# arpg/vicalib

Hardware: AMD Instinct MI355X
Metric: corner_residuals_per_sec (higher is better)
Workload: dtype f64

## Files before the change

vicalib_amd/csrc/vc_imu.hpp:

```cpp
#pragma once
#include "vc_math.hpp"

namespace vc {

struct D1 { double a, v; };
VC_HD D1 mk(double a, double v = 0.0) { D1 r; r.a = a; r.v = v; return r; }
VC_HD D1 operator+(D1 x, D1 y) { return mk(x.a + y.a, x.v + y.v); }
VC_HD D1 operator-(D1 x, D1 y) { return mk(x.a - y.a, x.v - y.v); }
VC_HD D1 operator-(D1 x) { return mk(-x.a, -x.v); }
VC_HD D1 operator*(D1 x, D1 y) { return mk(x.a * y.a, x.a * y.v + x.v * y.a); }
VC_HD D1 operator/(D1 x, D1 y) { const double inv = fast_rcp(y.a), q = x.a * inv; return mk(q, (x.v - q * y.v) * inv); }
VC_HD D1 operator+(D1 x, double s) { return mk(x.a + s, x.v); }
VC_HD D1 operator+(double s, D1 x) { return mk(x.a + s, x.v); }
VC_HD D1 operator-(D1 x, double s) { return mk(x.a - s, x.v); }
VC_HD D1 operator-(double s, D1 x) { return mk(s - x.a, -x.v); }
VC_HD D1 operator*(D1 x, double s) { return mk(x.a * s, x.v * s); }
VC_HD D1 operator*(double s, D1 x) { return mk(x.a * s, x.v * s); }
VC_HD D1 operator/(D1 x, double s) { const double inv = 1.0 / s; return mk(x.a * inv, x.v * inv); }
VC_HD D1 operator/(double s, D1 y) { const double inv = fast_rcp(y.a); return mk(s * inv, -s * inv * inv * y.v); }
VC_HD bool operator<(D1 x, double y) { return x.a < y; }
VC_HD bool operator>(D1 x, double y) { return x.a > y; }
VC_HD D1 sqrt(D1 x) { double s, is; fast_sqrt_rsqrt(x.a, &s, &is); return mk(s, 0.5 * x.v * is); }
VC_HD D1 sin(D1 x) { return mk(::sin(x.a), ::cos(x.a) * x.v); }
VC_HD D1 cos(D1 x) { return mk(::cos(x.a), -::sin(x.a) * x.v); }
// ... 229 lines not shown
  imu_integrate_pose(*s, k, dt * 0.5, &y);
  imu_pose_derivative(y, g_w, z0, z1, par, dt / 2.0, k);
  for (int i = 0; i < 9; ++i) ks[i] = ks[i] + 2.0 * k[i];
  imu_integrate_pose(*s, k, dt, &y);
  imu_pose_derivative(y, g_w, z0, z1, par, dt, k);
  for (int i = 0; i < 9; ++i) k[i] = ks[i] + k[i];
  imu_integrate_pose(*s, k, dt / 6.0, &y);
  *s = y;
}
template <class T> VC_HD void imu_rk4_step(PoseV<T>* s, const Meas<T>& z0, const Meas<T>& z1, const T* b, const T* sf, const T* g_w) {
  const ImuParamsPtr<T> par = {b, sf};
  imu_rk4_step_p(s, z0, z1, par, g_w);
}
template <class T> VC_HD void imu_gravity(const T* dir, T* out) {
  const double g = 9.8007;
  const T sp = sin(dir[0]), cp = cos(dir[0]), sq = sin(dir[1]), cq = cos(dir[1]);
  out[0] = (cp * sq) * (-g);
  out[1] = (-1.0 * sp) * (-g);
  out[2] = (cp * cq) * (-g);
}

VC_HD void imu_gravity_record(const double* gdir, double* rec9) {
  for (int c = 0; c < 2; ++c) {
    const D1 d[2] = {mk(gdir[0], c == 0 ? 1.0 : 0.0), mk(gdir[1], c == 1 ? 1.0 : 0.0)};
    D1 g[3];
    imu_gravity(d, g);
    for (int i = 0; i < 3; ++i) { rec9[i] = g[i].a; rec9[3 + 3 * c + i] = g[i].v; }
  }
}
template <class T>
VC_HD void imu_residual_tail(const PoseV<T>& s, const double* w_sqrt, int rotation_only, const T* T2, const T* v2, T* r) {
  T qc[4] = {-T2[0], -T2[1], -T2[2], T2[3]};
  T nt[3] = {T2[4] * -1.0, T2[5] * -1.0, T2[6] * -1.0}, ti[3];
  tq_rotate(qc, nt, ti);
  T rel[7], tr[3];
  tq_mul(s.q, qc, rel);
  const T nrm = sqrt(rel[0] * rel[0] + rel[1] * rel[1] + rel[2] * rel[2] + rel[3] * rel[3]);
  for (int i = 0; i < 4; ++i) rel[i] = rel[i] / nrm;
  tq_rotate(s.q, ti, tr);
  for (int i = 0; i < 3; ++i) rel[4 + i] = s.p[i] + tr[i];
  T raw[9];
  tse3_log(rel, raw);
  for (int i = 0; i < 3; ++i) raw[6 + i] = s.v[i] - v2[i];
  for (int j = 0; j < 9; ++j) {
    T acc = cst<T>(0.0);
    for (int i = 0; i < 9; ++i) acc = acc + raw[i] * w_sqrt[i * 9 + j];
    r[j] = acc;
  }
  if (rotation_only) for (int i = 0; i < 3; ++i) { r[i] = cst<T>(0.0); r[6 + i] = cst<T>(0.0); }
}

template <class T>
VC_HD void imu_residual(const ImuView& buf, double t_start, double t_end, const double* w_sqrt, int rotation_only,
                        const T* T2, const T* T1, const T* v2, const T* v1, const T* gdir, const T* b, const T* sf, T toff, T* r) {
  const ImuRange rg = imu_range(buf, t_start, t_end, val(toff));
  if (!rg.valid) { for (int i = 0; i < 9; ++i) r[i] = cst<T>(0.0); return; }
  T gw[3];
  imu_gravity(gdir, gw);
  PoseV<T> s;
  for (int i = 0; i < 4; ++i) s.q[i] = T1[i];
  for (int i = 0; i < 3; ++i) { s.p[i] = T1[4 + i]; s.v[i] = v1[i]; }
  const int n_meas = (rg.k1 - rg.k0 + 1) + 2;
  Meas<T> z0, z1;
  imu_range_get(buf, rg, toff, t_start, t_end, 0, &z0);
  for (int m = 1; m < n_meas; ++m) {
    imu_range_get(buf, rg, toff, t_start, t_end, m, &z1);
    imu_rk4_step(&s, z0, z1, b, sf, gw);
    z0 = z1;
  }
  imu_residual_tail(s, w_sqrt, rotation_only, T2, v2, r);
}

VC_HD void local_jac_se3(const double* x, double* J) {
  for (int i = 0; i < 42; ++i) J[i] = 0.0;
  const double q1 = x[0], q2 = x[1], q3 = x[2], q0 = x[3];
  J[0 * 6 + 3] = 0.5 * q0; J[0 * 6 + 4] = -0.5 * q3; J[0 * 6 + 5] = 0.5 * q2;
  J[1 * 6 + 3] = 0.5 * q3; J[1 * 6 + 4] = 0.5 * q0; J[1 * 6 + 5] = -0.5 * q1;
  J[2 * 6 + 3] = -0.5 * q2; J[2 * 6 + 4] = 0.5 * q1; J[2 * 6 + 5] = 0.5 * q0;
  J[3 * 6 + 3] = -0.5 * q1; J[3 * 6 + 4] = -0.5 * q2; J[3 * 6 + 5] = -0.5 * q3;
  J[4 * 6 + 0] = 1.0 - 2.0 * (q2 * q2 + q3 * q3); J[4 * 6 + 1] = 2.0 * (q1 * q2 - q0 * q3); J[4 * 6 + 2] = 2.0 * (q1 * q3 + q0 * q2);
  J[5 * 6 + 0] = 2.0 * (q1 * q2 + q0 * q3); J[5 * 6 + 1] = 1.0 - 2.0 * (q1 * q1 + q3 * q3); J[5 * 6 + 2] = 2.0 * (q2 * q3 - q0 * q1);
  J[6 * 6 + 0] = 2.0 * (q1 * q3 - q0 * q2); J[6 * 6 + 1] = 2.0 * (q2 * q3 + q0 * q1); J[6 * 6 + 2] = 1.0 - 2.0 * (q1 * q1 + q2 * q2);
}

VC_HD void imu_block_direction(const ImuView& buf, double t_start, double t_end, const double* w_sqrt, int rotation_only,
                               const double* T2, const double* T1, const double* v2, const double* v1, const double* gdir,
                               const double* b, const double* sf, double toff, int dir, double* r, double* dr) {
  D1 P[35];
  for (int i = 0; i < 7; ++i) { P[i] = mk(T2[i]); P[7 + i] = mk(T1[i]); }
  for (int i = 0; i < 3; ++i) { P[14 + i] = mk(v2[i]); P[17 + i] = mk(v1[i]); }
  P[20] = mk(gdir[0]); P[21] = mk(gdir[1]);
  for (int i = 0; i < 6; ++i) { P[22 + i] = mk(b[i]); P[28 + i] = mk(sf[i]); }
  P[34] = mk(toff);
  for (int i = 0; i < 35; ++i) P[i].v = (i == dir) ? 1.0 : 0.0;
  D1 res[9];
  imu_residual<D1>(buf, t_start, t_end, w_sqrt, rotation_only, P, P + 7, P + 14, P + 17, P + 20, P + 22, P + 28, P[34], res);
  for (int i = 0; i < 9; ++i) { r[i] = res[i].a; dr[i] = res[i].v; }
}

constexpr int kDeltaCols = 14;

template <class T> struct DeltaAcc { T q[4], p[3], v[3], t; };
template <class T> VC_HD void imu_delta_append(DeltaAcc<T>* A, const PoseV<T>& d, T dt) {
  T rp[3], rv[3], q[4];
  tq_rotate(A->q, d.p, rp);
  tq_rotate(A->q, d.v, rv);
  tq_mul(A->q, d.q, q);
  for (int i = 0; i < 3; ++i) {
    A->p[i] = (A->p[i] + A->v[i] * dt) + rp[i];
    A->v[i] = A->v[i] + rv[i];
  }
  for (int i = 0; i < 4; ++i) A->q[i] = q[i];
  A->t = A->t + dt;
}
template <class T> VC_HD void imu_delta_then(DeltaAcc<T>* a, const DeltaAcc<T>& x) {
  PoseV<T> d;
  for (int k = 0; k < 4; ++k) d.q[k] = x.q[k];
  for (int k = 0; k < 3; ++k) { d.p[k] = x.p[k]; d.v[k] = x.v[k]; }
  imu_delta_append(a, d, x.t);
}
template <class T> VC_HD void imu_delta_identity(DeltaAcc<T>* a) {
  for (int k = 0; k < 3; ++k) { a->q[k] = cst<T>(0.0); a->p[k] = cst<T>(0.0); a->v[k] = cst<T>(0.0); }
  a->q[3] = cst<T>(1.0); a->t = cst<T>(0.0);
}
constexpr int kBlockDeltaStride = kDeltaCols * 11;

VC_HD void so3_exp_jl(const double* w, double* q, double* A, double* B) {
  const double th2 = w[0] * w[0] + w[1] * w[1] + w[2] * w[2];
  double imag, real;
  tso3_exp_factors(th2, &imag, &real);
  q[0] = imag * w[0]; q[1] = imag * w[1]; q[2] = imag * w[2]; q[3] = real;
  const bool tiny = th2 < 1e-6;
  *A = 2.0 * imag * imag;
  *B = tiny ? 1.0 / 6.0 - th2 * (1.0 / 120.0) : (1.0 - 2.0 * imag * real) * fast_rcp(tiny ? 1.0 : th2);
}
VC_HD void cross3(const double* a, const double* b, double* o) {
  const double x = a[1] * b[2] - a[2] * b[1], y = a[2] * b[0] - a[0] * b[2], z = a[0] * b[1] - a[1] * b[0];
  o[0] = x; o[1] = y; o[2] = z;
}
VC_HD void so3_jl_apply(const double* w, double A, double B, const double* d, double* o) {
  double c1[3], c2[3];
  cross3(w, d, c1);
  cross3(w, c1, c2);
  for (int i = 0; i < 3; ++i) o[i] = d[i] + A * c1[i] + B * c2[i];
}
VC_HD void mat3_vec(const double* R, const double* v, double* o) {
  const double a = R[0] * v[0] + R[1] * v[1] + R[2] * v[2];
  const double b = R[3] * v[0] + R[4] * v[1] + R[5] * v[2];
  const double c = R[6] * v[0] + R[7] * v[1] + R[8] * v[2];
  o[0] = a; o[1] = b; o[2] = c;
}
struct IntervalDeltaT { DeltaAcc<double> d; double dth[3], dp[3], dv[3], dt; double ap[3], av[3]; };
constexpr int kDtDoubles = 27;
VC_HD void imu_delta_t_identity(IntervalDeltaT* X) {
  imu_delta_identity(&X->d);
  for (int i = 0; i < 3; ++i) { X->dth[i] = 0.0; X->dp[i] = 0.0; X->dv[i] = 0.0; X->ap[i] = 0.0; X->av[i] = 0.0; }
  X->dt = 0.0;
}
VC_HD void imu_interval_delta_t(const ImuView& buf, const ImuRange& rg, D1 off, double t_start, double t_end, int m, int n_int,
                                const double* b, const double* sf, int gsel, IntervalDeltaT* X) {
  imu_delta_t_identity(X);
  const int kk = gsel < 3 ? gsel : (gsel < 6 ? gsel - 3 : 0);
  const bool seeded = gsel < 6, scale = gsel >= 3;
  double u0[3], u1[3], a0[3], a1[3], du0[3], du1[3], da0[3], da1[3], h, dh;
  double c0, c1;
  {
    Meas<D1> z0, z1;
    for (int k = 0; k < 3; ++k) { z0.w[k] = z0.a[k] = z1.w[k] = z1.a[k] = mk(0.0); }
    z0.time = z1.time = mk(0.0);
    if (m <= n_int) { imu_range_get_flat(buf, rg, off, t_start, t_end, m - 1, &z0); imu_range_get_flat(buf, rg, off, t_start, t_end, m, &z1); }
    if (z1.time.a == z0.time.a) return;
    h = z1.time.a - z0.time.a; dh = z1.time.v - z0.time.v;
    for (int i = 0; i < 3; ++i) {
      const double s0 = (seeded && i == kk) ? (scale ? z0.w[i].a : 1.0) : 0.0, s1 = (seeded && i == kk) ? (scale ? z1.w[i].a : 1.0) : 0.0;
      u0[i] = z0.w[i].a * sf[i] + b[i]; du0[i] = z0.w[i].v * sf[i] + s0;
      u1[i] = z1.w[i].a * sf[i] + b[i]; du1[i] = z1.w[i].v * sf[i] + s1;
      a0[i] = z0.a[i].a * sf[3 + i] + b[3 + i]; da0[i] = z0.a[i].v * sf[3 + i];
      a1[i] = z1.a[i].a * sf[3 + i] + b[3 + i]; da1[i] = z1.a[i].v * sf[3 + i];
    }
    c0 = scale ? (kk == 0 ? z0.a[0].a : kk == 1 ? z0.a[1].a : z0.a[2].a) : 1.0;
    c1 = scale ? (kk == 0 ? z1.a[0].a : kk == 1 ? z1.a[1].a : z1.a[2].a) : 1.0;
  }
  const double hh = h * 0.5, h6 = h / 6.0, dhh = dh * 0.5, dh6 = dh / 6.0;
  const double cm = 0.5 * c0 + 0.5 * c1;
  double sw[3], sv[3], sp[3], dsw[3], dsv[3], dsp[3], cv[3], cp[3], phi[3], dphi[3];
  for (int i = 0; i < 3; ++i) {
    sw[i] = u0[i]; dsw[i] = du0[i]; sv[i] = a0[i]; dsv[i] = da0[i]; sp[i] = a0[i]; dsp[i] = da0[i];
    cv[i] = (i == kk) ? c0 : 0.0; cp[i] = cv[i];
    phi[i] = u0[i] * hh; dphi[i] = du0[i] * hh + u0[i] * dhh;
  }
  for (int stage = 2; stage <= 4; ++stage) {
    double q[4], A, B, R[9], dth[3], ug[3], ua[3], dug[3], dua[3], wk[3], ak[3], dwk[3], dak[3], t1[3], t2[3];
    so3_exp_jl(phi, q, &A, &B);
    quat_to_R(q, R);
    so3_jl_apply(phi, A, B, dphi, dth);
    for (int i = 0; i < 3; ++i) {
      if (stage < 4) { ug[i] = u0[i] * 0.5 + u1[i] * 0.5; ua[i] = a0[i] * 0.5 + a1[i] * 0.5; dug[i] = du0[i] * 0.5 + du1[i] * 0.5; dua[i] = da0[i] * 0.5 + da1[i] * 0.5; }
      else { ug[i] = u1[i]; ua[i] = a1[i]; dug[i] = du1[i]; dua[i] = da1[i]; }
    }
    mat3_vec(R, ug, wk); mat3_vec(R, ua, ak);
    cross3(dth, wk, t1); mat3_vec(R, dug, t2);
    for (int i = 0; i < 3; ++i) dwk[i] = t1[i] + t2[i];
    cross3(dth, ak, t1); mat3_vec(R, dua, t2);
    for (int i = 0; i < 3; ++i) dak[i] = t1[i] + t2[i];
    const double r[3] = {kk == 0 ? R[0] : kk == 1 ? R[1] : R[2], kk == 0 ? R[3] : kk == 1 ? R[4] : R[5], kk == 0 ? R[6] : kk == 1 ? R[7] : R[8]};
    const double wgt = stage < 4 ? 2.0 : 1.0, cc = stage < 4 ? cm : c1;
    for (int i = 0; i < 3; ++i) {
      sw[i] = sw[i] + wgt * wk[i]; dsw[i] = dsw[i] + wgt * dwk[i];
      sv[i] = sv[i] + wgt * ak[i]; dsv[i] = dsv[i] + wgt * dak[i];
      cv[i] = cv[i] + wgt * (cc * r[i]);
      if (stage < 4) { sp[i] = sp[i] + ak[i]; dsp[i] = dsp[i] + dak[i]; cp[i] = cp[i] + cc * r[i]; }
      const double hs = stage == 2 ? hh : h, dhs = stage == 2 ? dhh : dh;
      if (stage < 4) { phi[i] = wk[i] * hs; dphi[i] = dwk[i] * hs + wk[i] * dhs; }
    }
  }
  {
    double A, B;
    for (int i = 0; i < 3; ++i) { phi[i] = sw[i] * h6; dphi[i] = dsw[i] * h6 + sw[i] * dh6; }
    so3_exp_jl(phi, X->d.q, &A, &B);
    so3_jl_apply(phi, A, B, dphi, X->dth);
    const double hh6 = h * h6, dhh6 = 2.0 * h * dh6;
    for (int i = 0; i < 3; ++i) {
      X->d.v[i] = sv[i] * h6; X->dv[i] = dsv[i] * h6 + sv[i] * dh6;
      X->d.p[i] = sp[i] * hh6; X->dp[i] = dsp[i] * hh6 + sp[i] * dhh6;
      X->av[i] = cv[i] * h6; X->ap[i] = cp[i] * hh6;
    }
    X->d.t = h; X->dt = dh;
  }
}
VC_HD void imu_delta_t_then(IntervalDeltaT* A, const IntervalDeltaT& X) {
  double R[9], rp[3], rv[3], t1[3], t2[3], t3[3], q[4];
  quat_to_R(A->d.q, R);
  mat3_vec(R, X.d.p, rp); mat3_vec(R, X.d.v, rv);
  cross3(A->dth, rp, t1); mat3_vec(R, X.dp, t2);
  for (int i = 0; i < 3; ++i) A->dp[i] = ((A->dp[i] + A->dv[i] * X.d.t) + A->d.v[i] * X.dt) + (t1[i] + t2[i]);
  cross3(A->dth, rv, t1); mat3_vec(R, X.dv, t2);
  for (int i = 0; i < 3; ++i) A->dv[i] = A->dv[i] + (t1[i] + t2[i]);
  mat3_vec(R, X.dth, t3);
  for (int i = 0; i < 3; ++i) A->dth[i] = A->dth[i] + t3[i];
  A->dt = A->dt + X.dt;
  mat3_vec(R, X.ap, t1); mat3_vec(R, X.av, t2);
  for (int i = 0; i < 3; ++i) {
    A->ap[i] = (A->ap[i] + A->av[i] * X.d.t) + t1[i];
    A->av[i] = A->av[i] + t2[i];
  }
  for (int i = 0; i < 3; ++i) {
    A->d.p[i] = (A->d.p[i] + A->d.v[i] * X.d.t) + rp[i];
    A->d.v[i] = A->d.v[i] + rv[i];
  }
  quat_mul(A->d.q, X.d.q, q);
  for (int i = 0; i < 4; ++i) A->d.q[i] = q[i];
  A->d.t = A->d.t + X.d.t;
}
VC_HD int imu_group_dual_col(int g) { return g < 3 ? 1 + g : (g < 6 ? 4 + g : 13); }
VC_HD int imu_group_accel_col(int g) { return g < 3 ? 4 + g : 7 + g; }
VC_HD void imu_block_record_store(const IntervalDeltaT& X, int g, double* rec) {
  if (g > 6) return;
  double* cd = rec + imu_group_dual_col(g) * 11;
  const double hq[4] = {0.5 * X.dth[0], 0.5 * X.dth[1], 0.5 * X.dth[2], 0.0};
  double dq[4];
  quat_mul(hq, X.d.q, dq);
  for (int k = 0; k < 4; ++k) cd[k] = dq[k];
  for (int k = 0; k < 3; ++k) { cd[4 + k] = X.dp[k]; cd[7 + k] = X.dv[k]; }
  cd[10] = X.dt;
  if (g < 6) {
    double* ca = rec + imu_group_accel_col(g) * 11;
    for (int k = 0; k < 4; ++k) ca[k] = 0.0;
    for (int k = 0; k < 3; ++k) { ca[4 + k] = X.ap[k]; ca[7 + k] = X.av[k]; }
    ca[10] = 0.0;
  }
  if (g == 0) {
    for (int k = 0; k < 4; ++k) rec[k] = X.d.q[k];
    for (int k = 0; k < 3; ++k) { rec[4 + k] = X.d.p[k]; rec[7 + k] = X.d.v[k]; }
    rec[10] = X.d.t;
  }
}
inline int imu_block_delta_record(const ImuView& buf, double t_start, double t_end, double toff, const double* b, const double* sf,
                                  double* rec ) {
  const ImuRange rg = imu_range(buf, t_start, t_end, toff);
  if (!rg.valid) { rec[10] = -1.0; return 0; }
  const int n_int = (rg.k1 - rg.k0 + 1) + 1;
  for (int g = 0; g < 7; ++g) {
    const D1 offD = mk(toff, g == 6 ? 1.0 : 0.0);
    IntervalDeltaT carry;
    for (int base = 0; base < n_int; base += 16) {
      IntervalDeltaT X[8], Y[8];
      for (int l = 0; l < 8; ++l) {
        IntervalDeltaT second;
        imu_interval_delta_t(buf, rg, offD, t_start, t_end, base + 2 * l + 1, n_int, b, sf, g, &X[l]);
        imu_interval_delta_t(buf, rg, offD, t_start, t_end, base + 2 * l + 2, n_int, b, sf, g, &second);
        imu_delta_t_then(&X[l], second);
      }
      for (int n = 1; n < 8; n <<= 1) {
        for (int l = 0; l < 8; ++l) { Y[l] = X[l]; if (l >= n) { Y[l] = X[l - n]; imu_delta_t_then(&Y[l], X[l]); } }
        for (int l = 0; l < 8; ++l) X[l] = Y[l];
      }
      if (base == 0) carry = X[7]; else imu_delta_t_then(&carry, X[7]);
    }
    imu_block_record_store(carry, g, rec);
  }
  return 1;
}

VC_HD void imu_block_final_direction(int valid, const double* block_rec, const double* w_sqrt, int rotation_only, const double* T2,
                                     const double* T1, const double* v2, const double* v1, const double* grav9 , int col,
                                     double* r, double* dr) {
  if (!valid) { for (int i = 0; i < 9; ++i) { r[i] = 0.0; dr[i] = 0.0; } return; }
  const int dcol = (col >= 20) ? col - 19 : 0;
  D1 Q[4], P[3], V[3];
  double bd[11];
  for (int k = 0; k < 11; ++k) { const double d = block_rec[dcol * 11 + k]; bd[k] = dcol ? d : 0.0; }
  for (int k = 0; k < 4; ++k) Q[k] = mk(block_rec[k], bd[k]);
  for (int k = 0; k < 3; ++k) { P[k] = mk(block_rec[4 + k], bd[4 + k]); V[k] = mk(block_rec[7 + k], bd[7 + k]); }
  const D1 Tt = mk(block_rec[10], bd[10]);
  D1 T2D[7], v2D[3], gw[3], q0[4], p0[3], v0[3];
  {
    double J[42];
    local_jac_se3(T2, J);
    for (int i = 0; i < 7; ++i) {
      double sel = 0.0;
      for (int c = 0; c < 6; ++c) sel = (col == c) ? J[i * 6 + c] : sel;
      T2D[i] = mk(T2[i], sel);
    }
    local_jac_se3(T1, J);
    for (int i = 0; i < 7; ++i) {
      double sel = 0.0;
      for (int c = 0; c < 6; ++c) sel = (col == 9 + c) ? J[i * 6 + c] : sel;
      if (i < 4) q0[i] = mk(T1[i], sel); else p0[i - 4] = mk(T1[i], sel);
    }
  }
  for (int k = 0; k < 3; ++k) { v2D[k] = mk(v2[k], col == 6 + k ? 1.0 : 0.0); v0[k] = mk(v1[k], col == 15 + k ? 1.0 : 0.0); }
  for (int k = 0; k < 3; ++k) gw[k] = mk(grav9[k], col == 18 ? grav9[3 + k] : (col == 19 ? grav9[6 + k] : 0.0));
  PoseV<D1> x;
  D1 rp[3], rv[3];
  tq_rotate(q0, P, rp);
  tq_rotate(q0, V, rv);
  tq_mul(q0, Q, x.q);
  const D1 ht2 = 0.5 * (Tt * Tt);
  for (int i = 0; i < 3; ++i) {
    x.p[i] = ((p0[i] + v0[i] * Tt) - gw[i] * ht2) + rp[i];
    x.v[i] = (v0[i] - gw[i] * Tt) + rv[i];
  }
  D1 res[9];
  imu_residual_tail(x, w_sqrt, rotation_only, T2D, v2D, res);
  for (int i = 0; i < 9; ++i) { r[i] = res[i].a; dr[i] = res[i].v; }
}

}
```

vicalib_amd/csrc/vc_imu_kernels.hip:

```cpp
#include <hip/hip_runtime.h>
#include <algorithm>
#include <cstdlib>
#include "vc_math.hpp"
#include "vc_imu.hpp"
#include "vc_imu_weights.hpp"
#include "vc_device.h"
#include "vc_chain_order.hpp"
#include "vc_kutil.hpp"
#include "vc_reduced_tail.hpp"
#include "vc_shared_blocks.hpp"

namespace vc {

__device__ __forceinline__ ImuView imu_view(const DevView& v) { ImuView b = {v.imu_t, v.imu_w, v.imu_a, v.n_imu, v.imu_avg_dt}; return b; }

constexpr int kImuJacLds = 34 * 9 + 6;
struct SegTab {
  unsigned short v[kSegStride];
  constexpr SegTab() : v() { for (int e = 0; e < kSegLen; ++e) { int a = 0, b = 0; seg_entry(e, &a, &b); v[e] = (unsigned short)(a | (b << 8)); } }
};
__constant__ SegTab d_seg_tab = SegTab();
constexpr int kSegIters = (kSegLen + 31) / 32;
#ifndef VC_IJ_MFMA
#define VC_IJ_MFMA 1
#endif
struct SegInv {
  unsigned short v[9][64][4];
  constexpr SegInv() : v() {
    for (int t = 0; t < 9; ++t) for (int l = 0; l < 64; ++l) for (int g = 0; g < 4; ++g) v[t][l][g] = 0xffff;
    for (int e = 0; e < kSegLen; ++e) {
      int a = 0, b = 0; seg_entry(e, &a, &b);
      const int I = a / 16, J = b / 16, rt = a % 16;
      v[I * 3 + J][(rt % 4) * 16 + b % 16][rt / 4] = (unsigned short)e;
    }
  }
};
__constant__ SegInv d_seg_inv = SegInv();
#ifdef VC_IJ_STAMPS
#define IJSTAMP(i) do { if (blockIdx.x == 0 && threadIdx.x == 0) v.dbg[i] = (long long)__builtin_amdgcn_s_memrealtime(); } while (0)
#else
#define IJSTAMP(i) do { } while (0)
#endif
__global__ __launch_bounds__(256) void k_imu_jac(DevView v, int wr, int trial) {
  __shared__ double sh[8 * kImuJacLds];
  __shared__ double s_wq[8 * 84];
  IJSTAMP(0);
  if (trial && v.sync_seq > 0 && workgroup_pass_void(v)) return;
  const Ctrl* ct = v.ctrl;
  if (ct->done || (!trial && !ct->need_lin)) {
    if (trial && v.final_wait > 0 && threadIdx.x == 0) __hip_atomic_fetch_add(v.sync_flags + 11, 1LL, __ATOMIC_RELAXED, __HIP_MEMORY_SCOPE_AGENT);
    return;
  }
  const int wave = threadIdx.x >> 6, lane = threadIdx.x & 63;
  const int half = lane >> 5, l = lane & 31;
  const int n_blocks = v.n_frames - 1;
  const int s_raw = (blockIdx.x * 4 + wave) * 2 + half;
  const bool exists = s_raw < n_blocks;
  const int s = exists ? s_raw : n_blocks - 1;
  const int cur = trial ? 1 - ct->cur : ct->cur, j = s + 1;
  double* Jl = sh + (wave * 2 + half) * kImuJacLds;
  const double* T2 = v.poses[cur] + (size_t)j * kPoseStride;
  const double* T1 = v.poses[cur] + (size_t)(j - 1) * kPoseStride;
  const double* v2 = v.vel[cur] + (size_t)j * 4;
  const double* v1 = v.vel[cur] + (size_t)(j - 1) * 4;
  const double* wq_g = v.wsqrtb[wr] + (size_t)s * 81;
  double* wq = s_wq + (wave * 2 + half) * 84;
  {
    double t3[3];
#pragma unroll
    for (int t = 0; t < 3; ++t) { const int idx = l + 32 * t; t3[t] = wq_g[idx < 81 ? idx : 0]; }
#pragma unroll
    for (int t = 0; t < 3; ++t) { const int idx = l + 32 * t; if (idx < 81) wq[idx] = t3[t]; }
  }
  const double* brec = v.imu_delta_blk + (size_t)s * kBlockDeltaStride;
  double r[9], dr[9];
  const int col = (l < 6) ? l : (l < 30 ? l + 3 : -1);
  const bool valid = brec[10] >= 0.0;
#if VC_IJ_MFMA
  unsigned long long seg_at[9];
#pragma unroll
  for (int t = 0; t < 9; ++t) seg_at[t] = t == 6 ? ~0ull : *reinterpret_cast<const unsigned long long*>(&d_seg_inv.v[t][lane][0]);
#else
  int seg_ab[kSegIters];
#pragma unroll
  for (int it = 0; it < kSegIters; ++it) { const int e = l + 32 * it; seg_ab[it] = d_seg_tab.v[e < kSegLen ? e : 0]; }
#endif
  wave_lds_sync();
  IJSTAMP(1);
  imu_block_final_direction(valid, brec, wq, v.rotation_only, T2, T1, v2, v1, v.imu_grav + cur * 16, col, r, dr);
  IJSTAMP(2);
  if (col >= 0) {
#pragma unroll
    for (int k = 0; k < 9; ++k) Jl[col * 9 + k] = dr[k];
  }
  if (l < 3) {
#pragma unroll
    for (int k = 0; k < 9; ++k) {
      const bool zeroed = v.rotation_only && (k < 3 || k >= 6);
      Jl[(6 + l) * 9 + k] = (valid && !zeroed) ? -wq[(6 + l) * 9 + k] : 0.0;
    }
  }
  if (l == 31) {
#pragma unroll
    for (int k = 0; k < 9; ++k) Jl[33 * 9 + k] = r[k];
  }
  wave_lds_sync();
  double ss = 0.0;
#pragma unroll
  for (int k = 0; k < 9; ++k) ss += r[k] * r[k];
  double rho, rho1;
  loss_cauchy100(ss, &rho, &rho1);
  const double w = ct->imu_mult * rho1;
  if (trial) {
    __shared__ double s_cost[8];
    if (l == 0) s_cost[wave * 2 + half] = exists ? ct->imu_mult * rho : 0.0;
    __syncthreads();
    if (threadIdx.x == 0) {
      const double wc = ((s_cost[0] + s_cost[1]) + (s_cost[2] + s_cost[3])) + ((s_cost[4] + s_cost[5]) + (s_cost[6] + s_cost[7]));
      if (v.final_wait > 0) {
        __hip_atomic_store(v.wg_imu_trial + blockIdx.x, wc, __ATOMIC_RELAXED, __HIP_MEMORY_SCOPE_AGENT);
        __builtin_amdgcn_s_waitcnt(0);
        __hip_atomic_fetch_add(v.sync_flags + 4, 1LL, __ATOMIC_RELAXED, __HIP_MEMORY_SCOPE_AGENT);
      } else v.wg_imu_trial[blockIdx.x] = wc;
    }
  }
  IJSTAMP(3);
  const bool counted2 = trial && v.final_wait > 0;
#if VC_IJ_MFMA
  {
    const int i16 = lane & 15, kq = lane >> 4;
#pragma unroll
    for (int h = 0; h < 2; ++h) {
      if (!__builtin_amdgcn_readlane((int)exists, 32 * h)) continue;
      const double wh = readlane_f64(w, 32 * h);
      const int sb = __builtin_amdgcn_readlane(s, 32 * h);
      const double* Jb = sh + (wave * 2 + h) * kImuJacLds;
      double op[3][3];
#pragma unroll
      for (int T = 0; T < 3; ++T)
#pragma unroll
        for (int ks = 0; ks < 3; ++ks) {
          const int c = 16 * T + i16, rr = 4 * ks + kq;
          const bool in = c < 34 && rr < 9;
          const double x = Jb[in ? c * 9 + rr : 0];
          op[T][ks] = in ? x : 0.0;
        }
      double* rec = v.segb[cur] + (size_t)sb * kSegStride;
#pragma unroll
      for (int I = 0; I < 3; ++I)
#pragma unroll
        for (int J = 0; J < 3; ++J) {
          if (I == 2 && J == 0) continue;
          v4d acc = (v4d){0.0, 0.0, 0.0, 0.0};
#pragma unroll
          for (int ks = 0; ks < 3; ++ks) acc = __builtin_amdgcn_mfma_f64_16x16x4f64(op[I][ks], op[J][ks], acc, 0, 0, 0);
          const unsigned long long at = seg_at[I * 3 + J];
#pragma unroll
          for (int g = 0; g < 4; ++g) {
            const unsigned e = (unsigned)(at >> (16 * g)) & 0xffffu;
            if (e != 0xffffu) { if (counted2) __hip_atomic_store(rec + e, wh * acc[g], __ATOMIC_RELAXED, __HIP_MEMORY_SCOPE_AGENT); else rec[e] = wh * acc[g]; }
          }
        }
    }
    if (exists && l == 0) { if (counted2) __hip_atomic_store(v.seg_costb[cur] + s, ct->imu_mult * rho, __ATOMIC_RELAXED, __HIP_MEMORY_SCOPE_AGENT); else v.seg_costb[cur][s] = ct->imu_mult * rho; }
  }
#else
  if (exists) {
  double* rec = v.segb[cur] + (size_t)s * kSegStride;
#pragma unroll
  for (int it = 0; it < kSegIters; ++it) {
    const int e = l + 32 * it;
    const int ab = seg_ab[it], a = ab & 255, bb = ab >> 8;
    double acc = 0.0;
#pragma unroll
    for (int k = 0; k < 9; ++k) acc += Jl[a * 9 + k] * Jl[bb * 9 + k];
    if (e < kSegLen) { if (counted2) __hip_atomic_store(rec + e, w * acc, __ATOMIC_RELAXED, __HIP_MEMORY_SCOPE_AGENT); else rec[e] = w * acc; }
  }
  if (l == 0) { if (counted2) __hip_atomic_store(v.seg_costb[cur] + s, ct->imu_mult * rho, __ATOMIC_RELAXED, __HIP_MEMORY_SCOPE_AGENT); else v.seg_costb[cur][s] = ct->imu_mult * rho; }
  }
#endif
  if (counted2) {
    __builtin_amdgcn_s_waitcnt(0);
    __syncthreads();
    if (threadIdx.x == 0) __hip_atomic_fetch_add(v.sync_flags + 11, 1LL, __ATOMIC_RELAXED, __HIP_MEMORY_SCOPE_AGENT);
  }
  IJSTAMP(4);
}

constexpr int kWLds = 184;
constexpr int kWPose = 88, kWVel = 104, kWImu = 108, kWSig = 128;

template <int CTRL> __device__ __forceinline__ double dpp_f64(double old, double x) {
  const int lo = __builtin_amdgcn_update_dpp(__double2loint(old), __double2loint(x), CTRL, 0xf, 0xf, false);
  const int hi = __builtin_amdgcn_update_dpp(__double2hiint(old), __double2hiint(x), CTRL, 0xf, 0xf, false);
  return __hiloint2double(hi, lo);
}
template <int N> __device__ __forceinline__ double row_shr(double old, double x) { return dpp_f64<0x110 + N>(old, x); }
template <int N> __device__ __forceinline__ double row_shl(double old, double x) { return dpp_f64<0x100 + N>(old, x); }
template <int CTRL> __device__ __forceinline__ double dpp_perm(double x) {
  const int lo = __builtin_amdgcn_mov_dpp(__double2loint(x), CTRL, 0xf, 0xf, false);
  const int hi = __builtin_amdgcn_mov_dpp(__double2hiint(x), CTRL, 0xf, 0xf, false);
  return __hiloint2double(hi, lo);
}
template <int CTRL, int N> __device__ __forceinline__ void row_add_level(double* x) {
  double y[N];
#pragma unroll
  for (int e = 0; e < N; ++e) y[e] = dpp_perm<CTRL>(x[e]);
#pragma unroll
  for (int e = 0; e < N; ++e) x[e] += y[e];
}
template <int N> __device__ __forceinline__ void row_allsum_n(double* x) {
  row_add_level<0xB1, N>(x);
  row_add_level<0x4E, N>(x);
  row_add_level<0x141, N>(x);
  row_add_level<0x140, N>(x);
}
__device__ __forceinline__ double shfl16(double x, int src) { return __shfl(x, src, 16); }
__device__ __forceinline__ void delta_identity(DeltaAcc<double>* a) {
#pragma unroll
  for (int k = 0; k < 3; ++k) { a->q[k] = 0.0; a->p[k] = 0.0; a->v[k] = 0.0; }
  a->q[3] = 1.0; a->t = 0.0;
}
__device__ __forceinline__ void delta_then(DeltaAcc<double>* a, const DeltaAcc<double>& x) {
  PoseV<double> d;
#pragma unroll
  for (int k = 0; k < 4; ++k) d.q[k] = x.q[k];
#pragma unroll
  for (int k = 0; k < 3; ++k) { d.p[k] = x.p[k]; d.v[k] = x.v[k]; }
  imu_delta_append(a, d, x.t);
}
template <int N> __device__ __forceinline__ void delta_scan_level(DeltaAcc<double>* X, int c) {
  DeltaAcc<double> A;
#pragma unroll
  for (int k = 0; k < 4; ++k) A.q[k] = row_shr<N>(X->q[k], X->q[k]);
#pragma unroll
  for (int k = 0; k < 3; ++k) { A.p[k] = row_shr<N>(X->p[k], X->p[k]); A.v[k] = row_shr<N>(X->v[k], X->v[k]); }
  A.t = row_shr<N>(X->t, X->t);
  delta_then(&A, *X);
  if (c >= N) *X = A;
}
template <int N> __device__ __forceinline__ void map_scan_level(double* S) {
  double B[kWMapF], O[kWMapF];
  w_map_identity(B);
#pragma unroll
  for (int e = 0; e < kWMapF; ++e) B[e] = row_shl<N>(B[e], S[e]);
  w_map_compose(B, S, O);
#pragma unroll
  for (int e = 0; e < kWMapF; ++e) S[e] = O[e];
}

__device__ __forceinline__ ImuRange imu_range_lanes(const ImuView& b, double t0, double t1, double off, int lane) {
  ImuRange r; r.valid = 0; r.k0 = 0; r.k1 = -1; r.i0 = r.i1 = 0; r.first_end = r.last_end = 0;
  if (b.n < 2) return r;
  const bool odd = lane & 1;
  int idx, endc, le;
  imu_element_index(b, odd ? t1 : t0, off, &idx, &endc, &le);
  const int idx_o = __shfl_xor(idx, 1, 64), endc_o = __shfl_xor(endc, 1, 64), le_o = __shfl_xor(le, 1, 64);
  r.valid = (t0 >= b.t[0] + off && t0 <= b.t[b.n - 1] + off) ? 1 : 0;
  r.i0 = odd ? idx_o : idx; r.first_end = odd ? endc_o : endc;
  r.i1 = odd ? idx : idx_o; r.last_end = odd ? endc : endc_o;
  r.k0 = r.i0 + 1;
  r.k1 = odd ? le : le_o;
  if (r.k1 < r.i0) r.k1 = r.i0;
  return r;
}

__device__ __forceinline__ void delta_t_pack(const IntervalDeltaT& X, double* f) {
#pragma unroll
  for (int k = 0; k < 4; ++k) f[k] = X.d.q[k];
#pragma unroll
  for (int k = 0; k < 3; ++k) { f[4 + k] = X.d.p[k]; f[7 + k] = X.d.v[k]; f[11 + k] = X.dth[k]; f[14 + k] = X.dp[k]; f[17 + k] = X.dv[k]; f[21 + k] = X.ap[k]; f[24 + k] = X.av[k]; }
  f[10] = X.d.t; f[20] = X.dt;
}
__device__ __forceinline__ void delta_t_unpack(const double* f, IntervalDeltaT* X) {
#pragma unroll
  for (int k = 0; k < 4; ++k) X->d.q[k] = f[k];
#pragma unroll
  for (int k = 0; k < 3; ++k) { X->d.p[k] = f[4 + k]; X->d.v[k] = f[7 + k]; X->dth[k] = f[11 + k]; X->dp[k] = f[14 + k]; X->dv[k] = f[17 + k]; X->ap[k] = f[21 + k]; X->av[k] = f[24 + k]; }
  X->d.t = f[10]; X->dt = f[20];
}
template <int N> __device__ __forceinline__ void delta_t_scan_level(IntervalDeltaT* X, int l) {
  double f[kDtDoubles];
  delta_t_pack(*X, f);
#pragma unroll
  for (int k = 0; k < kDtDoubles; ++k) f[k] = row_shr<N>(f[k], f[k]);
  IntervalDeltaT A;
  delta_t_unpack(f, &A);
  imu_delta_t_then(&A, *X);
  if (l >= N) *X = A;
}
#ifdef VC_IB_STAMPS
#define IBSTAMP(i) do { if (blockIdx.x == gridDim.x / 2 && threadIdx.x == 0) v.dbg[i] = (long long)__builtin_amdgcn_s_memrealtime(); } while (0)
#else
#define IBSTAMP(i) do { } while (0)
#endif
#ifndef VC_IMU_BLOCK_WAVES
#define VC_IMU_BLOCK_WAVES 2
#endif
#ifdef VC_IMU_BLOCK_EU
__global__ __launch_bounds__(256) __attribute__((amdgpu_waves_per_eu(VC_IMU_BLOCK_EU, VC_IMU_BLOCK_EU))) void k_imu_block(DevView v, int trial) {
#else
__global__ __launch_bounds__(256, VC_IMU_BLOCK_WAVES) void k_imu_block(DevView v, int trial) {
#endif
  __shared__ double s_carry[32 * kDtDoubles];
  __shared__ double s_park[256 * (kDtDoubles - 11)];
  __shared__ double s_parkv[4 * 8 * 11];
  IBSTAMP(0);
  if (trial && v.sync_seq > 0 && workgroup_pass_void(v)) return;
  const int lane = threadIdx.x & 63, wave = __builtin_amdgcn_readfirstlane(threadIdx.x >> 6);
  const int g = lane >> 3, l = lane & 7;
  const int n_blocks = v.n_frames - 1;
  const int s_raw = blockIdx.x * 4 + wave;
  const int s = s_raw < n_blocks ? s_raw : n_blocks - 1;
  const double toff0 = v.imus[0][14], toff1 = v.imus[1][14];
  const double t_start = v.frame_time[s], t_end = v.frame_time[s + 1];
  const Ctrl* ct = v.ctrl;
  const int c_done = ct->done, c_need = ct->need_lin, c_cur = ct->cur;
  if (c_done || (!trial && !c_need)) return;
  IBSTAMP(1);
  const int cur = trial ? 1 - c_cur : c_cur;
  const double* im = v.imus[cur];
  const double toff = cur ? toff1 : toff0;
  const ImuView buf = imu_view(v);
  ImuRange rg = imu_range_lanes(buf, t_start, t_end, toff, lane);
  rg.valid = __builtin_amdgcn_readfirstlane(rg.valid); rg.i0 = __builtin_amdgcn_readfirstlane(rg.i0); rg.i1 = __builtin_amdgcn_readfirstlane(rg.i1);
  rg.k0 = __builtin_amdgcn_readfirstlane(rg.k0); rg.k1 = __builtin_amdgcn_readfirstlane(rg.k1);
  rg.first_end = __builtin_amdgcn_readfirstlane(rg.first_end); rg.last_end = __builtin_amdgcn_readfirstlane(rg.last_end);
  double* rec = v.imu_delta_blk + (size_t)s * kBlockDeltaStride;
  IBSTAMP(2);
  if (rg.valid) {
    const int n_int = (rg.k1 - rg.k0 + 1) + 1;
    const int gsel = g < 7 ? g : 6;
    double* cr = s_carry + (threadIdx.x >> 3) * kDtDoubles;
    IntervalDeltaT X;
#pragma unroll 1
    for (int base = 0; base < n_int; base += 16) {
      {
        IntervalDeltaT Y;
        double* pk = s_park + threadIdx.x;
        double* pv = s_parkv + (wave * 8 + l) * 11;
#pragma unroll 1
        for (int half = 0; half < 2; ++half) {
          int gs = gsel;
          asm volatile("" : "+v"(gs));
          imu_interval_delta_t(buf, rg, mk(toff, gs == 6 ? 1.0 : 0.0), t_start, t_end, base + 2 * l + 1 + half, n_int, im + 2, im + 8, gs, &Y);
          IBSTAMP(3 + half);
          if (half == 0) {
            double f[kDtDoubles];
            delta_t_pack(Y, f);
#pragma unroll
            for (int k = 11; k < kDtDoubles; ++k) pk[(k - 11) * 256] = f[k];
            if (g == 0) {
#pragma unroll
              for (int k = 0; k < 11; ++k) pv[k] = f[k];
            }
          }
        }
        wave_lds_sync_local();
        double f[kDtDoubles];
#pragma unroll
        for (int k = 0; k < 11; ++k) f[k] = pv[k];
#pragma unroll
        for (int k = 11; k < kDtDoubles; ++k) f[k] = pk[(k - 11) * 256];
        delta_t_unpack(f, &X);
        wave_lds_sync_local();
        imu_delta_t_then(&X, Y);
      }
      IBSTAMP(5);
      delta_t_scan_level<1>(&X, l); delta_t_scan_level<2>(&X, l); delta_t_scan_level<4>(&X, l);
      IBSTAMP(6);
      if (l == 7) {
        if (base > 0) {
          IntervalDeltaT A;
          double f[kDtDoubles];
#pragma unroll
          for (int k = 0; k < kDtDoubles; ++k) f[k] = cr[k];
          delta_t_unpack(f, &A);
          imu_delta_t_then(&A, X);
          X = A;
        }
        if (base + 16 < n_int) {
          double f[kDtDoubles];
          delta_t_pack(X, f);
#pragma unroll
          for (int k = 0; k < kDtDoubles; ++k) cr[k] = f[k];
        }
      }
    }
    if (l == 7 && s_raw < n_blocks) imu_block_record_store(X, g, rec);
    IBSTAMP(7);
  } else if (lane == 0 && s_raw < n_blocks) rec[10] = -1.0;
  if (blockIdx.x == 0 && threadIdx.x == 63) imu_gravity_record(im, v.imu_grav + cur * 16);
  if (trial && v.block_wait > 0 && blockIdx.x == 0 && threadIdx.x == 0) spin_until_flag<false>(v, 2, v.block_wait);
}

#ifdef VC_W_STAMPS
#define WSTAMP(i) do { if (blockIdx.x == 0 && threadIdx.x == 0) v.dbg[i] = (long long)__builtin_amdgcn_s_memrealtime(); } while (0)
#else
#define WSTAMP(i) do { } while (0)
#endif
__global__ __launch_bounds__(64) void k_imu_weights(DevView v, int wr) {
  __shared__ __attribute__((aligned(16))) double w_lds[4 * kWLds];
  const Ctrl* ct = v.ctrl;
  const int lane = threadIdx.x;
  const int grp = lane >> 4, c = lane & 15;
  const int n_blocks = v.n_frames - 1;
  const int s_raw = blockIdx.x * 4 + grp;
  const bool exists = s_raw < n_blocks;
  const int s = exists ? s_raw : n_blocks - 1;
  double* L = w_lds + grp * kWLds;
  if (v.sync_seq > 0) { const long long m = sync_marked(v); if (m != 0 && m <= v.sync_seq) return; }
  if (ct->done == kDoneSyncTimeout) return;
  if (ct->done || !v.weights_on) {
    if (exists) for (int e = c; e < 81; e += 16) v.wsqrtb[1 - wr][(size_t)s * 81 + e] = v.wsqrtb[wr][(size_t)s * 81 + e];
    return;
  }
  WSTAMP(0);
  const int j = s + 1;
  {
    const double p0 = v.poses[0][(size_t)(j - 1) * kPoseStride + c], p1 = v.poses[1][(size_t)(j - 1) * kPoseStride + c];
    const double u0 = v.vel[0][(size_t)(j - 1) * 4 + (c & 3)], u1 = v.vel[1][(size_t)(j - 1) * 4 + (c & 3)];
    const int ci = c < 15 ? c : 14;
    const double i0 = v.imus[0][ci], i1 = v.imus[1][ci];
    const bool one = ct->cur != 0;
    L[kWPose + c] = one ? p1 : p0;
    if (c < 4) L[kWVel + c] = one ? u1 : u0;
    if (c < 15) L[kWImu + c] = one ? i1 : i0;
  }
  const double t_start = v.frame_time[j - 1], t_end = v.frame_time[j];
  wave_lds_sync();
  double b[6], sf[6];
#pragma unroll
  for (int i = 0; i < 6; ++i) { b[i] = L[kWImu + 2 + i]; sf[i] = L[kWImu + 8 + i]; }
  const double toff = L[kWImu + 14];
  const ImuView buf = imu_view(v);
  const ImuRange rg = imu_range_lanes(buf, t_start, t_end, toff, lane);
  const bool live = exists && rg.valid;
  const double sg2 = v.gyro_sigma * v.gyro_sigma, sa2 = v.accel_sigma * v.accel_sigma;
  const int n_int = live ? (rg.k1 - rg.k0 + 1) + 1 : 0;
  int n_max = n_int;
#pragma unroll
  for (int o = 32; o >= 16; o >>= 1) n_max = max(n_max, __shfl_xor(n_max, o, 64));
  DeltaAcc<double> carry;
  delta_identity(&carry);
  const double g0[3] = {0.0, 0.0, 0.0};
  WSTAMP(1);
#pragma unroll 1
  for (int base = 0; base < n_max; base += 16) {
    const int m = base + c + 1;
    Meas<double> z0, z1;
#pragma unroll
    for (int k = 0; k < 3; ++k) { z0.w[k] = z0.a[k] = z1.w[k] = z1.a[k] = 0.0; }
    z0.time = z1.time = 0.0;
    if (m <= n_int) { imu_range_get_flat(buf, rg, toff, t_start, t_end, m - 1, &z0); imu_range_get_flat(buf, rg, toff, t_start, t_end, m, &z1); }
    const bool act = z1.time != z0.time;
    WSTAMP(2);
    DeltaAcc<double> X;
    {
      PoseV<double> d;
#pragma unroll
      for (int k = 0; k < 3; ++k) { d.q[k] = 0.0; d.p[k] = 0.0; d.v[k] = 0.0; }
      d.q[3] = 1.0;
      imu_rk4_step(&d, z0, z1, b, sf, g0);
#pragma unroll
      for (int k = 0; k < 4; ++k) X.q[k] = d.q[k];
#pragma unroll
      for (int k = 0; k < 3; ++k) { X.p[k] = d.p[k]; X.v[k] = d.v[k]; }
      X.t = z1.time - z0.time;
    }
    WSTAMP(3);
    delta_scan_level<1>(&X, c); delta_scan_level<2>(&X, c); delta_scan_level<4>(&X, c); delta_scan_level<8>(&X, c);
    double q_st[4];
    {
      double qe[4], ident[4] = {0.0, 0.0, 0.0, 1.0};
#pragma unroll
      for (int k = 0; k < 4; ++k) ident[k] = row_shr<1>(ident[k], X.q[k]);
      quat_mul(carry.q, ident, qe);
      const double q1[4] = {L[kWPose + 0], L[kWPose + 1], L[kWPose + 2], L[kWPose + 3]};
      quat_mul(q1, qe, q_st);
      DeltaAcc<double> Tt;
#pragma unroll
// ... 2621 lines not shown
```

Baseline: 2.167 billion.

## Preload IMU inputs into registers and stage segment records in LDS for coalesced stores

New measurement: 2.173 billion (median of 4 runs). Within noise of the previous version (+0.3%).

```diff
diff --git a/vicalib_amd/csrc/vc_imu.hpp b/vicalib_amd/csrc/vc_imu.hpp
--- a/vicalib_amd/csrc/vc_imu.hpp
+++ b/vicalib_amd/csrc/vc_imu.hpp
@@ -555,17 +555,18 @@
   return 1;
 }
 
-VC_HD void imu_block_final_direction(int valid, const double* block_rec, const double* w_sqrt, int rotation_only, const double* T2,
-                                     const double* T1, const double* v2, const double* v1, const double* grav9 , int col,
-                                     double* r, double* dr) {
+VC_HD int imu_block_dcol(int col) { return (col >= 20) ? col - 19 : 0; }
+VC_HD void imu_block_final_direction_regs(int valid, const double* rec0, const double* recd, const double* w_sqrt, int rotation_only,
+                                          const double* T2, const double* T1, const double* v2, const double* v1,
+                                          const double* grav9 , int col, double* r, double* dr) {
   if (!valid) { for (int i = 0; i < 9; ++i) { r[i] = 0.0; dr[i] = 0.0; } return; }
-  const int dcol = (col >= 20) ? col - 19 : 0;
+  const int dcol = imu_block_dcol(col);
   D1 Q[4], P[3], V[3];
   double bd[11];
-  for (int k = 0; k < 11; ++k) { const double d = block_rec[dcol * 11 + k]; bd[k] = dcol ? d : 0.0; }
-  for (int k = 0; k < 4; ++k) Q[k] = mk(block_rec[k], bd[k]);
-  for (int k = 0; k < 3; ++k) { P[k] = mk(block_rec[4 + k], bd[4 + k]); V[k] = mk(block_rec[7 + k], bd[7 + k]); }
-  const D1 Tt = mk(block_rec[10], bd[10]);
+  for (int k = 0; k < 11; ++k) bd[k] = dcol ? recd[k] : 0.0;
+  for (int k = 0; k < 4; ++k) Q[k] = mk(rec0[k], bd[k]);
+  for (int k = 0; k < 3; ++k) { P[k] = mk(rec0[4 + k], bd[4 + k]); V[k] = mk(rec0[7 + k], bd[7 + k]); }
+  const D1 Tt = mk(rec0[10], bd[10]);
   D1 T2D[7], v2D[3], gw[3], q0[4], p0[3], v0[3];
   {
     double J[42];
@@ -598,5 +599,17 @@
   imu_residual_tail(x, w_sqrt, rotation_only, T2D, v2D, res);
   for (int i = 0; i < 9; ++i) { r[i] = res[i].a; dr[i] = res[i].v; }
 }
-
-}
+VC_HD void imu_block_final_direction(int valid, const double* block_rec, const double* w_sqrt, int rotation_only, const double* T2,
+                                     const double* T1, const double* v2, const double* v1, const double* grav9 , int col,
+                                     double* r, double* dr) {
+  if (!valid) { for (int i = 0; i < 9; ++i) { r[i] = 0.0; dr[i] = 0.0; } return; }
+  const int dcol = imu_block_dcol(col);
+  double rec0[11], recd[11], a2[7], a1[7], b2[3], b1[3], g9[9];
+  for (int k = 0; k < 11; ++k) { rec0[k] = block_rec[k]; recd[k] = block_rec[dcol * 11 + k]; }
+  for (int k = 0; k < 7; ++k) { a2[k] = T2[k]; a1[k] = T1[k]; }
+  for (int k = 0; k < 3; ++k) { b2[k] = v2[k]; b1[k] = v1[k]; }
+  for (int k = 0; k < 9; ++k) g9[k] = grav9[k];
+  imu_block_final_direction_regs(valid, rec0, recd, w_sqrt, rotation_only, a2, a1, b2, b1, g9, col, r, dr);
+}
+
+}
diff --git a/vicalib_amd/csrc/vc_imu_kernels.hip b/vicalib_amd/csrc/vc_imu_kernels.hip
--- a/vicalib_amd/csrc/vc_imu_kernels.hip
+++ b/vicalib_amd/csrc/vc_imu_kernels.hip
@@ -36,6 +36,8 @@
   }
 };
 __constant__ SegInv d_seg_inv = SegInv();
+constexpr int kImuRecLds = kSegLen + 1;
+constexpr int kImuRecStores = (kSegLen + 63) / 64;
 #ifdef VC_IJ_STAMPS
 #define IJSTAMP(i) do { if (blockIdx.x == 0 && threadIdx.x == 0) v.dbg[i] = (long long)__builtin_amdgcn_s_memrealtime(); } while (0)
 #else
@@ -45,9 +47,19 @@
   __shared__ double sh[8 * kImuJacLds];
   __shared__ double s_wq[8 * 84];
   IJSTAMP(0);
-  if (trial && v.sync_seq > 0 && workgroup_pass_void(v)) return;
+  const bool ask_void = trial && v.sync_seq > 0;
+  long long marked = 0;
+  if (ask_void && threadIdx.x == 0) marked = sync_marked(v);
   const Ctrl* ct = v.ctrl;
-  if (ct->done || (!trial && !ct->need_lin)) {
+  const int c_done = ct->done, c_cur = ct->cur, c_need_lin = ct->need_lin;
+  const double imu_mult = ct->imu_mult;
+  if (ask_void) {
+    __shared__ int s_void;
+    if (threadIdx.x == 0) s_void = (marked != 0 && marked <= v.sync_seq) ? 1 : 0;
+    __syncthreads();
+    if (s_void != 0) return;
+  }
+  if (c_done || (!trial && !c_need_lin)) {
     if (trial && v.final_wait > 0 && threadIdx.x == 0) __hip_atomic_fetch_add(v.sync_flags + 11, 1LL, __ATOMIC_RELAXED, __HIP_MEMORY_SCOPE_AGENT);
     return;
   }
@@ -57,7 +69,7 @@
   const int s_raw = (blockIdx.x * 4 + wave) * 2 + half;
   const bool exists = s_raw < n_blocks;
   const int s = exists ? s_raw : n_blocks - 1;
-  const int cur = trial ? 1 - ct->cur : ct->cur, j = s + 1;
+  const int cur = trial ? 1 - c_cur : c_cur, j = s + 1;
   double* Jl = sh + (wave * 2 + half) * kImuJacLds;
   const double* T2 = v.poses[cur] + (size_t)j * kPoseStride;
   const double* T1 = v.poses[cur] + (size_t)(j - 1) * kPoseStride;
@@ -65,30 +77,42 @@
   const double* v1 = v.vel[cur] + (size_t)(j - 1) * 4;
   const double* wq_g = v.wsqrtb[wr] + (size_t)s * 81;
   double* wq = s_wq + (wave * 2 + half) * 84;
+  const double* brec = v.imu_delta_blk + (size_t)s * kBlockDeltaStride;
+  const double* grav = v.imu_grav + cur * 16;
+  double r[9], dr[9];
+  const int col = (l < 6) ? l : (l < 30 ? l + 3 : -1);
+  double rec0[11], recd[11], T2r[7], T1r[7], v2r[3], v1r[3], g9[9];
   {
     double t3[3];
 #pragma unroll
     for (int t = 0; t < 3; ++t) { const int idx = l + 32 * t; t3[t] = wq_g[idx < 81 ? idx : 0]; }
+    const int dcol = imu_block_dcol(col);
+#pragma unroll
+    for (int k = 0; k < 11; ++k) { rec0[k] = brec[k]; recd[k] = brec[dcol * 11 + k]; }
+#pragma unroll
+    for (int k = 0; k < 7; ++k) { T2r[k] = T2[k]; T1r[k] = T1[k]; }
+#pragma unroll
+    for (int k = 0; k < 3; ++k) { v2r[k] = v2[k]; v1r[k] = v1[k]; }
+#pragma unroll
+    for (int k = 0; k < 9; ++k) g9[k] = grav[k];
 #pragma unroll
     for (int t = 0; t < 3; ++t) { const int idx = l + 32 * t; if (idx < 81) wq[idx] = t3[t]; }
   }
-  const double* brec = v.imu_delta_blk + (size_t)s * kBlockDeltaStride;
-  double r[9], dr[9];
-  const int col = (l < 6) ? l : (l < 30 ? l + 3 : -1);
-  const bool valid = brec[10] >= 0.0;
+  const bool valid = rec0[10] >= 0.0;
+#if !VC_IJ_MFMA
+  int seg_ab[kSegIters];
+#pragma unroll
+  for (int it = 0; it < kSegIters; ++it) { const int e = l + 32 * it; seg_ab[it] = d_seg_tab.v[e < kSegLen ? e : 0]; }
+#endif
+  wave_lds_sync();
+  IJSTAMP(1);
+  imu_block_final_direction_regs(valid, rec0, recd, wq, v.rotation_only, T2r, T1r, v2r, v1r, g9, col, r, dr);
+  IJSTAMP(2);
 #if VC_IJ_MFMA
   unsigned long long seg_at[9];
 #pragma unroll
   for (int t = 0; t < 9; ++t) seg_at[t] = t == 6 ? ~0ull : *reinterpret_cast<const unsigned long long*>(&d_seg_inv.v[t][lane][0]);
-#else
-  int seg_ab[kSegIters];
-#pragma unroll
-  for (int it = 0; it < kSegIters; ++it) { const int e = l + 32 * it; seg_ab[it] = d_seg_tab.v[e < kSegLen ? e : 0]; }
-#endif
-  wave_lds_sync();
-  IJSTAMP(1);
-  imu_block_final_direction(valid, brec, wq, v.rotation_only, T2, T1, v2, v1, v.imu_grav + cur * 16, col, r, dr);
-  IJSTAMP(2);
+#endif
   if (col >= 0) {
 #pragma unroll
     for (int k = 0; k < 9; ++k) Jl[col * 9 + k] = dr[k];
@@ -104,16 +128,16 @@
 #pragma unroll
     for (int k = 0; k < 9; ++k) Jl[33 * 9 + k] = r[k];
   }
-  wave_lds_sync();
+  wave_lds_sync_local();
   double ss = 0.0;
 #pragma unroll
   for (int k = 0; k < 9; ++k) ss += r[k] * r[k];
   double rho, rho1;
   loss_cauchy100(ss, &rho, &rho1);
-  const double w = ct->imu_mult * rho1;
+  const double w = imu_mult * rho1;
   if (trial) {
     __shared__ double s_cost[8];
-    if (l == 0) s_cost[wave * 2 + half] = exists ? ct->imu_mult * rho : 0.0;
+    if (l == 0) s_cost[wave * 2 + half] = exists ? imu_mult * rho : 0.0;
     __syncthreads();
     if (threadIdx.x == 0) {
       const double wc = ((s_cost[0] + s_cost[1]) + (s_cost[2] + s_cost[3])) + ((s_cost[4] + s_cost[5]) + (s_cost[6] + s_cost[7]));
@@ -128,12 +152,14 @@
   const bool counted2 = trial && v.final_wait > 0;
 #if VC_IJ_MFMA
   {
+    __shared__ double s_rec[4 * kImuRecLds];
     const int i16 = lane & 15, kq = lane >> 4;
+    double* img = s_rec + wave * kImuRecLds;
+    double out[2][kImuRecStores];
 #pragma unroll
     for (int h = 0; h < 2; ++h) {
       if (!__builtin_amdgcn_readlane((int)exists, 32 * h)) continue;
       const double wh = readlane_f64(w, 32 * h);
-      const int sb = __builtin_amdgcn_readlane(s, 32 * h);
       const double* Jb = sh + (wave * 2 + h) * kImuJacLds;
       double op[3][3];
 #pragma unroll
@@ -145,7 +171,6 @@
           const double x = Jb[in ? c * 9 + rr : 0];
           op[T][ks] = in ? x : 0.0;
         }
-      double* rec = v.segb[cur] + (size_t)sb * kSegStride;
 #pragma unroll
       for (int I = 0; I < 3; ++I)
 #pragma unroll
@@ -158,11 +183,26 @@
 #pragma unroll
           for (int g = 0; g < 4; ++g) {
             const unsigned e = (unsigned)(at >> (16 * g)) & 0xffffu;
-            if (e != 0xffffu) { if (counted2) __hip_atomic_store(rec + e, wh * acc[g], __ATOMIC_RELAXED, __HIP_MEMORY_SCOPE_AGENT); else rec[e] = wh * acc[g]; }
+            if (e != 0xffffu) img[e] = wh * acc[g];
           }
         }
-    }
-    if (exists && l == 0) { if (counted2) __hip_atomic_store(v.seg_costb[cur] + s, ct->imu_mult * rho, __ATOMIC_RELAXED, __HIP_MEMORY_SCOPE_AGENT); else v.seg_costb[cur][s] = ct->imu_mult * rho; }
+      wave_lds_sync_local();
+#pragma unroll
+      for (int k = 0; k < kImuRecStores; ++k) { const int e = lane + 64 * k; out[h][k] = img[e < kSegLen ? e : 0]; }
+      wave_lds_sync_local();
+    }
+#pragma unroll
+    for (int h = 0; h < 2; ++h) {
+      if (!__builtin_amdgcn_readlane((int)exists, 32 * h)) continue;
+      const int sb = __builtin_amdgcn_readlane(s, 32 * h);
+      double* rec = v.segb[cur] + (size_t)sb * kSegStride;
+#pragma unroll
+      for (int k = 0; k < kImuRecStores; ++k) {
+        const int e = lane + 64 * k;
+        if (e < kSegLen) { if (counted2) __hip_atomic_store(rec + e, out[h][k], __ATOMIC_RELAXED, __HIP_MEMORY_SCOPE_AGENT); else rec[e] = out[h][k]; }
+      }
+    }
+    if (exists && l == 0) { if (counted2) __hip_atomic_store(v.seg_costb[cur] + s, imu_mult * rho, __ATOMIC_RELAXED, __HIP_MEMORY_SCOPE_AGENT); else v.seg_costb[cur][s] = imu_mult * rho; }
   }
 #else
   if (exists) {
@@ -176,7 +216,7 @@
     for (int k = 0; k < 9; ++k) acc += Jl[a * 9 + k] * Jl[bb * 9 + k];
     if (e < kSegLen) { if (counted2) __hip_atomic_store(rec + e, w * acc, __ATOMIC_RELAXED, __HIP_MEMORY_SCOPE_AGENT); else rec[e] = w * acc; }
   }
-  if (l == 0) { if (counted2) __hip_atomic_store(v.seg_costb[cur] + s, ct->imu_mult * rho, __ATOMIC_RELAXED, __HIP_MEMORY_SCOPE_AGENT); else v.seg_costb[cur][s] = ct->imu_mult * rho; }
+  if (l == 0) { if (counted2) __hip_atomic_store(v.seg_costb[cur] + s, imu_mult * rho, __ATOMIC_RELAXED, __HIP_MEMORY_SCOPE_AGENT); else v.seg_costb[cur][s] = imu_mult * rho; }
   }
 #endif
   if (counted2) {
```
